# RomanBresson/KAGNN

Hardware: AMD Instinct MI355X
Metric: edges/sec KAN-GIN fwd+bwd, hidden=64 grid=5, 1M-node synthetic; HBM % peak (higher is better)
Workload: dtype f32 (fp16 hi/lo split operands, fp32 accumulate)

## Files before the change

### kagnn_amd/csrc/aggregate.hip

```cpp
#include "common.h"
#include "host.h"

namespace kagnn {


__device__ __forceinline__ float4 ld4(const float* p) { return *reinterpret_cast<const float4*>(p); }
__device__ __forceinline__ void fma4(float4& a, float w, const float4& v) {
    a.x = fmaf(w, v.x, a.x); a.y = fmaf(w, v.y, a.y); a.z = fmaf(w, v.z, a.z); a.w = fmaf(w, v.w, a.w);
}

__device__ __forceinline__ float edge_w(const AggArgs& a, int e, int j, long i) {
    float w = a.ew ? a.ew[e] : 1.0f;
    if (a.in_scale) w *= a.in_scale[j];
    if (a.skip_self && j == (int)i) w = 0.0f;
    return w;
}

__device__ __forceinline__ void stats_products(const AggArgs& a, long row, int c4, const float4& o, float4& pa, float4& pb) {
    const float4 y = ld4(a.st_y + row * a.st_ldy + c4), m = ld4(a.st_mean + c4), q = ld4(a.st_rstd + c4);
    pa = o;
    pb = make_float4(o.x * ((y.x - m.x) * q.x), o.y * ((y.y - m.y) * q.y), o.z * ((y.z - m.z) * q.z), o.w * ((y.w - m.w) * q.w));
}

template <int LPR, bool STATS, bool LEAN>
__device__ __forceinline__ void agg_rows_v4_body(const AggArgs& args) {
    AggArgs a = args;
    if constexpr (LEAN) {
        a.ew = nullptr; a.in_scale = nullptr; a.out_scale = nullptr; a.bias = nullptr; a.skip_self = 0;
        a.col_scale = nullptr; a.col_shift = nullptr;
    }
    const unsigned wg = (LEAN ? a.wg0 : 0u) + (blockIdx.x & 7) * (gridDim.x >> 3) + (blockIdx.x >> 3);
    const long gid = (wg * 256L + threadIdx.x) / LPR;
    const int c4 = (threadIdx.x % LPR) * 4;
    const bool live = gid < a.N && c4 < a.F;
    if (!STATS && !live) return;
    float4 pa = make_float4(0.f, 0.f, 0.f, 0.f), pb = pa;
    if (live) {
        const int s = a.rowptr[gid], t = a.rowptr[gid + 1];
        const bool hub = (t - s) > a.hub_threshold;
        float4 acc = ld4(a.x + gid * a.ldx + c4);
        const float sw = a.self_scale * (a.in_scale ? a.in_scale[gid] : 1.0f);
        acc.x *= sw; acc.y *= sw; acc.z *= sw; acc.w *= sw;
        if (!hub) {
            int e = s;
            for (; e + 4 <= t; e += 4) {
                const int j0 = a.col[e], j1 = a.col[e + 1], j2 = a.col[e + 2], j3 = a.col[e + 3];
                const float4 v0 = ld4(a.x + (long)j0 * a.ldx + c4);
                const float4 v1 = ld4(a.x + (long)j1 * a.ldx + c4);
                const float4 v2 = ld4(a.x + (long)j2 * a.ldx + c4);
                const float4 v3 = ld4(a.x + (long)j3 * a.ldx + c4);
                fma4(acc, edge_w(a, e, j0, gid), v0);
                fma4(acc, edge_w(a, e + 1, j1, gid), v1);
                fma4(acc, edge_w(a, e + 2, j2, gid), v2);
                fma4(acc, edge_w(a, e + 3, j3, gid), v3);
            }
            for (; e < t; ++e) {
                const int j = a.col[e];
                fma4(acc, edge_w(a, e, j, gid), ld4(a.x + (long)j * a.ldx + c4));
            }
        }
        const float os = a.out_scale ? a.out_scale[gid] : 1.0f;
        float4 b = make_float4(0.f, 0.f, 0.f, 0.f);
        if (a.bias) b = ld4(a.bias + c4);
        float4 o = make_float4(fmaf(os, acc.x, b.x), fmaf(os, acc.y, b.y), fmaf(os, acc.z, b.z), fmaf(os, acc.w, b.w));
        if (a.col_scale) {
            const float4 cs = ld4(a.col_scale + c4), ch = ld4(a.col_shift + c4);
            const float cnt = (float)(t - s) + a.self_scale;
            o.x = fmaf(cs.x, o.x, cnt * ch.x); o.y = fmaf(cs.y, o.y, cnt * ch.y);
            o.z = fmaf(cs.z, o.z, cnt * ch.z); o.w = fmaf(cs.w, o.w, cnt * ch.w);
        }
        if (a.addend && !hub) {
            const float4 d = ld4(a.addend + gid * a.lda + c4);
            o.x += d.x; o.y += d.y; o.z += d.z; o.w += d.w;
        }
        *reinterpret_cast<float4*>(a.out + gid * a.ldo + c4) = o;
        if (STATS && !hub) stats_products(a, gid, c4, o, pa, pb);
    }
    if constexpr (STATS) {
        __shared__ float4 s_a[256], s_b[256];
        s_a[threadIdx.x] = pa; s_b[threadIdx.x] = pb;
        __syncthreads();
        if (threadIdx.x < LPR && c4 < a.F && wg * 256L < a.N * LPR) {
            constexpr int R = 256 / LPR;
#pragma unroll 4
            for (int k = 1; k < R; ++k) {
                const float4 u = s_a[k * LPR + threadIdx.x], v = s_b[k * LPR + threadIdx.x];
                pa.x += u.x; pa.y += u.y; pa.z += u.z; pa.w += u.w;
                pb.x += v.x; pb.y += v.y; pb.z += v.z; pb.w += v.w;
            }
            *reinterpret_cast<float4*>(a.st_partial + (wg * 2L + 0) * a.F + c4) = pa;
            *reinterpret_cast<float4*>(a.st_partial + (wg * 2L + 1) * a.F + c4) = pb;
        }
    }
}

template <int LPR, bool STATS = false>
__global__ __launch_bounds__(256) void agg_rows_v4_kernel(AggArgs a) { agg_rows_v4_body<LPR, STATS, false>(a); }

template <int LPR>
__global__ __launch_bounds__(256) void agg_rows_v4_corun_kernel(AggArgs a) { agg_rows_v4_body<LPR, false, true>(a); }

template <int LPR>
__global__ __launch_bounds__(256) void agg_rows_ep_kernel(AggArgs a) {
    constexpr int EP = 16 / LPR;
    const long gid = (blockIdx.x * 256L + threadIdx.x) >> 4;
    const int l16 = threadIdx.x & 15, cg = l16 % LPR, eg = l16 / LPR;
    const int c4 = cg * 4;
    const bool live = gid < a.N && c4 < a.F;
    const long row = min(gid, a.N - 1);
    const int cc = live ? c4 : 0;
    const int s = a.rowptr[row], t = a.rowptr[row + 1];
    const bool hub = (t - s) > a.hub_threshold;
    float4 acc = make_float4(0.f, 0.f, 0.f, 0.f);
    if (!hub) {
        int e = s + eg;
        for (; e + EP < t; e += 2 * EP) {
            const int j0 = a.col[e], j1 = a.col[e + EP];
            const float4 v0 = ld4(a.x + (long)j0 * a.ldx + cc);
            const float4 v1 = ld4(a.x + (long)j1 * a.ldx + cc);
            fma4(acc, edge_w(a, e, j0, row), v0);
            fma4(acc, edge_w(a, e + EP, j1, row), v1);
        }
        if (e < t) {
            const int j = a.col[e];
            fma4(acc, edge_w(a, e, j, row), ld4(a.x + (long)j * a.ldx + cc));
        }
    }
#pragma unroll
    for (int o = LPR; o < 16; o <<= 1) {
        acc.x += __shfl_xor(acc.x, o); acc.y += __shfl_xor(acc.y, o);
        acc.z += __shfl_xor(acc.z, o); acc.w += __shfl_xor(acc.w, o);
    }
    if (live && eg == 0) {
        const float sw = a.self_scale * (a.in_scale ? a.in_scale[row] : 1.0f);
        const float4 xs = ld4(a.x + row * a.ldx + c4);
        const float os = a.out_scale ? a.out_scale[row] : 1.0f;
        float4 b = make_float4(0.f, 0.f, 0.f, 0.f);
        if (a.bias) b = ld4(a.bias + c4);
        float4 o = make_float4(fmaf(os, fmaf(sw, xs.x, acc.x), b.x), fmaf(os, fmaf(sw, xs.y, acc.y), b.y),
                               fmaf(os, fmaf(sw, xs.z, acc.z), b.z), fmaf(os, fmaf(sw, xs.w, acc.w), b.w));
        if (a.col_scale) {
            const float4 cs = ld4(a.col_scale + c4), ch = ld4(a.col_shift + c4);
            const float cnt = (float)(t - s) + a.self_scale;
            o.x = fmaf(cs.x, o.x, cnt * ch.x); o.y = fmaf(cs.y, o.y, cnt * ch.y);
            o.z = fmaf(cs.z, o.z, cnt * ch.z); o.w = fmaf(cs.w, o.w, cnt * ch.w);
        }
        if (a.addend && !hub) {
            const float4 d = ld4(a.addend + row * a.lda + c4);
            o.x += d.x; o.y += d.y; o.z += d.z; o.w += d.w;
        }
        *reinterpret_cast<float4*>(a.out + row * a.ldo + c4) = o;
    }
}

template <int LPR>
__global__ __launch_bounds__(256) void agg_hub_v4_kernel(AggArgs a, const int* __restrict__ seg,
                                                         float* __restrict__ part, int ldp) {
    __shared__ float4 s_part[256];
    const int row = seg[3 * blockIdx.x], e0 = seg[3 * blockIdx.x + 1], e1 = seg[3 * blockIdx.x + 2];
    constexpr int G = 256 / LPR;
    const int g = threadIdx.x / LPR, lg = threadIdx.x % LPR, c4 = lg * 4;
    float4 acc = make_float4(0.f, 0.f, 0.f, 0.f);
    if (c4 < a.F) {
        int e = e0 + g;
        for (; e + 3 * G < e1; e += 4 * G) {
            const int j0 = a.col[e], j1 = a.col[e + G], j2 = a.col[e + 2 * G], j3 = a.col[e + 3 * G];
            const float4 v0 = ld4(a.x + (long)j0 * a.ldx + c4);
            const float4 v1 = ld4(a.x + (long)j1 * a.ldx + c4);
            const float4 v2 = ld4(a.x + (long)j2 * a.ldx + c4);
            const float4 v3 = ld4(a.x + (long)j3 * a.ldx + c4);
            fma4(acc, edge_w(a, e, j0, row), v0);
            fma4(acc, edge_w(a, e + G, j1, row), v1);
            fma4(acc, edge_w(a, e + 2 * G, j2, row), v2);
            fma4(acc, edge_w(a, e + 3 * G, j3, row), v3);
        }
        for (; e < e1; e += G) {
            const int j = a.col[e];
            fma4(acc, edge_w(a, e, j, row), ld4(a.x + (long)j * a.ldx + c4));
        }
    }
    s_part[threadIdx.x] = acc;
    __syncthreads();
    if (g == 0 && c4 < a.F) {
#pragma unroll 8
        for (int k = 1; k < G; ++k) {
            const float4 p = s_part[k * LPR + lg];
            acc.x += p.x; acc.y += p.y; acc.z += p.z; acc.w += p.w;
        }
        *reinterpret_cast<float4*>(part + (long)blockIdx.x * ldp + c4) = acc;
    }
}

template <int LPR, bool STATS = false>
__global__ __launch_bounds__(256) void agg_hub_merge_kernel(AggArgs a, const int* __restrict__ seg, long nseg,
                                                            const float* __restrict__ part, int ldp, long st_row0 = 0) {
    __shared__ float4 s_part[256];
// ... 148 lines not shown
}

__global__ __launch_bounds__(256) void embedding_fwd_kernel(const int64_t* __restrict__ idx, long stride, long N,
                                                            const float* __restrict__ table, int V, int F,
                                                            float* __restrict__ out, long ldo, int accumulate) {
    const long i = blockIdx.x * 4L + (threadIdx.x >> 6);
    if (i >= N) return;
    const int lane = threadIdx.x & 63;
    const int64_t v = idx[i * stride];
    const bool ok = v >= 0 && v < V;
    for (int f = lane; f < F; f += 64) {
        const float t = ok ? table[v * F + f] : __builtin_nanf("");
        out[i * ldo + f] = accumulate ? out[i * ldo + f] + t : t;
    }
}

constexpr int kEmbRows = 128;
template <int WAVES>
__global__ __launch_bounds__(64 * WAVES) void embedding_bwd_partial_kernel(const int64_t* __restrict__ idx, long stride, long N,
                                                                           const float* __restrict__ g, long ldg, int V, int F,
                                                                           float* __restrict__ partial) {
    extern __shared__ float s_acc[];
    const int lane = threadIdx.x & 63, wave = __builtin_amdgcn_readfirstlane(threadIdx.x >> 6), f = blockIdx.y * 64 + lane;
    float* acc = s_acc + (size_t)wave * V * 64;
    for (int k = lane; k < V * 64; k += 64) acc[k] = 0.0f;
    __builtin_amdgcn_wave_barrier();
    constexpr int RPW = kEmbRows / WAVES;
    const long r0 = ((long)blockIdx.x * WAVES + wave) * RPW, r1 = min(N, r0 + RPW);
    const bool col_ok = f < F;
    const int fc = min(f, F - 1);
    for (long i0 = r0; i0 < r1; i0 += 16) {
        int64_t iv[16];
        float gv[16];
#pragma unroll
        for (int u = 0; u < 16; ++u) iv[u] = idx[min(i0 + u, r1 - 1) * stride];
#pragma unroll
        for (int u = 0; u < 16; ++u) gv[u] = g[min(i0 + u, r1 - 1) * ldg + fc];
#pragma unroll
        for (int u = 0; u < 16; ++u) {
            const bool hit = i0 + u < r1 && iv[u] >= 0 && iv[u] < V;
            const float val = col_ok ? gv[u] : 0.0f;
            if (hit) acc[(int)iv[u] * 64 + lane] += val;
        }
    }
    __syncthreads();
    for (int k = threadIdx.x; k < V * 64; k += 64 * WAVES) {
        const int v = k >> 6, ff = blockIdx.y * 64 + (k & 63);
        float a = s_acc[k];
#pragma unroll
        for (int w = 1; w < WAVES; ++w) a += s_acc[(size_t)w * V * 64 + k];
        if (ff < F) partial[((long)blockIdx.x * V + v) * F + ff] = a;
    }
}

__global__ __launch_bounds__(256) void embedding_bwd_reduce_kernel(const float* __restrict__ partial, int nb, int V, int F,
                                                                   float* __restrict__ g_table) {
    __shared__ float s_part[8][32];
    const int e = threadIdx.x & 31, sub = threadIdx.x >> 5;
    const long per = (long)V * F, k = blockIdx.x * 32L + e;
    const int chunk = (nb + 7) / 8, b0 = sub * chunk, b1 = min(nb, b0 + chunk);
    float a = 0.0f;
    if (k < per) {
        int b = b0;
        for (; b + 8 <= b1; b += 8) {
            float t[8];
#pragma unroll
            for (int u = 0; u < 8; ++u) t[u] = partial[(b + u) * per + k];
#pragma unroll
            for (int u = 0; u < 8; ++u) a += t[u];
        }
        for (; b < b1; ++b) a += partial[b * per + k];
    }
    s_part[sub][e] = a;
    __syncthreads();
    if (sub == 0 && k < per) {
        float t = s_part[0][e];
#pragma unroll
        for (int q = 1; q < 8; ++q) t += s_part[q][e];
        g_table[k] = t;
    }
}

int embedding_fwd(const int64_t* idx, long stride, long N, const float* table, int V, int F, float* out, long ldo, int accumulate,
                  hipStream_t st) {
    if (N == 0) return KAGNN_OK;
    embedding_fwd_kernel<<<cdiv(N, 4), 256, 0, st>>>(idx, stride, N, table, V, F, out, ldo, accumulate);
    KAGNN_LAUNCH_CHECK();
    return KAGNN_OK;
}

size_t embedding_bwd_ws_bytes(long N, int V, int F) { return (size_t)cdiv(max(N, 1L), kEmbRows) * V * F * sizeof(float); }

int embedding_bwd(const int64_t* idx, long stride, long N, const float* g, long ldg, int V, int F, float* g_table, float* ws,
                  size_t ws_bytes, hipStream_t st) {
    if (V == 0) return KAGNN_OK;
    if (V > 512) return fail(KAGNN_ERR_UNSUPPORTED, "%s: tables of at most 512 rows (the categorical encoders of the graph-level models)", "embedding_bwd");
    if (ws_bytes < embedding_bwd_ws_bytes(N, V, F)) return fail(KAGNN_ERR_ARG, "%s: workspace too small", "embedding_bwd");
    const size_t tbl = (size_t)V * 64 * sizeof(float);
    const int waves = 4 * tbl <= 64 * 1024 ? 4 : 2 * tbl <= 128 * 1024 ? 2 : 1;
    const int nb = cdiv(max(N, 1L), (long)kEmbRows);
    const size_t lds = waves * tbl;
    if (lds > 64 * 1024) {
        static unsigned long long configured = 0;
        if (auto first_use_ = first_use_on_this_device(configured)) {
            KAGNN_HIP(hipFuncSetAttribute((const void*)embedding_bwd_partial_kernel<1>, hipFuncAttributeMaxDynamicSharedMemorySize, 128 * 1024 + 1024));
            KAGNN_HIP(hipFuncSetAttribute((const void*)embedding_bwd_partial_kernel<2>, hipFuncAttributeMaxDynamicSharedMemorySize, 128 * 1024 + 1024));
        }
    }
    const dim3 grid((unsigned)nb, (unsigned)cdiv(F, 64));
    if (waves == 4) embedding_bwd_partial_kernel<4><<<grid, 256, lds, st>>>(idx, stride, N, g, ldg, V, F, ws);
    else if (waves == 2) embedding_bwd_partial_kernel<2><<<grid, 128, lds, st>>>(idx, stride, N, g, ldg, V, F, ws);
    else embedding_bwd_partial_kernel<1><<<grid, 64, lds, st>>>(idx, stride, N, g, ldg, V, F, ws);
    KAGNN_LAUNCH_CHECK();
    embedding_bwd_reduce_kernel<<<cdiv((long)V * F, 32), 256, 0, st>>>(ws, nb, V, F, g_table);
    KAGNN_LAUNCH_CHECK();
    return KAGNN_OK;
}

static bool vec4_ok(const AggArgs& a) {
    auto al = [](const void* p) { return (reinterpret_cast<uintptr_t>(p) & 15) == 0; };
    return a.F % 4 == 0 && a.F <= 256 && a.ldx % 4 == 0 && a.ldo % 4 == 0 && al(a.x) && al(a.out) &&
           (!a.bias || al(a.bias)) && (!a.addend || (al(a.addend) && a.lda % 4 == 0)) &&
           (!a.col_scale || (al(a.col_scale) && al(a.col_shift)));
}

size_t aggregate_ws_bytes(long num_hub_seg, int F) { return (size_t)num_hub_seg * (size_t)((F + 3) & ~3) * sizeof(float); }

int aggregate_hub_rows(const AggArgs& a, const int* hub_seg, long num_hub_seg, float* ws, size_t ws_bytes, hipStream_t st) {
    if (num_hub_seg <= 0) return KAGNN_OK;
    const int ldp = (a.F + 3) & ~3;
    if ((size_t)num_hub_seg * ldp * sizeof(float) > ws_bytes) return fail(KAGNN_ERR_ARG, "%s: workspace too small", "aggregate_hub_rows");
#define HUBS(LPR)                                                                                   \
    {                                                                                               \
        agg_hub_v4_kernel<LPR><<<(unsigned)num_hub_seg, 256, 0, st>>>(a, hub_seg, ws, ldp);         \
        KAGNN_LAUNCH_CHECK();                                                                       \
        agg_hub_merge_kernel<LPR><<<(unsigned)num_hub_seg, 256, 0, st>>>(a, hub_seg, num_hub_seg, ws, ldp); \
        KAGNN_LAUNCH_CHECK();                                                                       \
    }
    if (a.F <= 4) HUBS(1) else if (a.F <= 8) HUBS(2) else if (a.F <= 16) HUBS(4) else if (a.F <= 32) HUBS(8)
    else if (a.F <= 64) HUBS(16) else if (a.F <= 128) HUBS(32) else HUBS(64)
#undef HUBS
    return KAGNN_OK;
}

static int stats_lpr(int F) { return F <= 32 ? 8 : F <= 64 ? 16 : F <= 128 ? 32 : 64; }
bool aggregate_stats_ok(const AggArgs& a) {
    auto al = [](const void* p) { return (reinterpret_cast<uintptr_t>(p) & 15) == 0; };
    return vec4_ok(a) && a.F > 16 && a.st_y && a.st_mean && a.st_rstd && a.st_partial && a.st_ldy % 4 == 0 && al(a.st_y) &&
           al(a.st_mean) && al(a.st_rstd) && al(a.st_partial);
}
long aggregate_stats_rows(long N, int F, long num_hub_seg) { return (long)cdiv(N * stats_lpr(F), 256) + (num_hub_seg > 0 ? num_hub_seg : 0); }

bool aggregate_corun_ok(const AggArgs& a) {
    return vec4_ok(a) && a.F > 32 && a.F <= 64 && !a.ew && !a.in_scale && !a.out_scale && !a.bias && !a.skip_self && !a.col_scale && !a.st_partial;
}

int aggregate_sum(const AggArgs& a, const int* hub_seg, long num_hub_seg, float* ws, size_t ws_bytes, hipStream_t st, const AggCorun* corun) {
    if (a.N == 0) return KAGNN_OK;
    if (corun && !(aggregate_corun_ok(a) && corun->head_pct >= 0 && corun->head_pct < 100 && corun->side_done))
        return fail(KAGNN_ERR_ARG, "%s: the co-run launch does not cover this call", "aggregate_sum");
    const bool stats = a.st_partial != nullptr;
    if (stats && !aggregate_stats_ok(a)) return fail(KAGNN_ERR_UNSUPPORTED, "%s: column statistics need 16-byte aligned fp32 rows of 17..256 columns", "aggregate_sum");
    if (!vec4_ok(a)) {
        AggArgs b = a;
        b.hub_threshold = 0x7fffffff;
        dim3 grid((unsigned)a.N, cdiv(a.F, 256));
        agg_rows_generic_kernel<<<grid, 256, 0, st>>>(b);
        KAGNN_LAUNCH_CHECK();
        return KAGNN_OK;
    }
    AggArgs b = a;
    if (num_hub_seg == 0 || hub_seg == nullptr) b.hub_threshold = 0x7fffffff;
    const int ldp = (a.F + 3) & ~3;
    if (b.hub_threshold != 0x7fffffff && (ws == nullptr || ws_bytes < aggregate_ws_bytes(num_hub_seg, a.F)))
        return fail(KAGNN_ERR_ARG, "%s: workspace too small for the hub segments (see kagnn_aggregate_workspace_bytes)", "aggregate_sum");
#define HUBS(LPR, ST)                                                                               \
    if (b.hub_threshold != 0x7fffffff) {                                                            \
        agg_hub_v4_kernel<LPR><<<(unsigned)num_hub_seg, 256, 0, st>>>(b, hub_seg, ws, ldp);         \
        KAGNN_LAUNCH_CHECK();                                                                       \
        agg_hub_merge_kernel<LPR, ST><<<(unsigned)num_hub_seg, 256, 0, st>>>(b, hub_seg, num_hub_seg, ws, ldp, (long)cdiv(a.N * LPR, 256)); \
        KAGNN_LAUNCH_CHECK();                                                                       \
    }
#define AGG_ROWS_GRID(threads) (cdiv(cdiv((threads), 256), 8) * 8)
#define ROWS(LPR)                                                                     \
    {                                                                                 \
        if (stats) {                                                                  \
            agg_rows_v4_kernel<LPR, true><<<AGG_ROWS_GRID(a.N * LPR), 256, 0, st>>>(b);   \
            KAGNN_LAUNCH_CHECK();                                                     \
            HUBS(LPR, true)                                                           \
        } else {                                                                      \
            if (corun && LPR == 16) {         \
                const unsigned total = AGG_ROWS_GRID(a.N * LPR);       \
                const unsigned head = (unsigned)((unsigned long)total * (unsigned)corun->head_pct / 100) & ~7u; \
                if (head) {                                                           \
                    agg_rows_v4_corun_kernel<16><<<head, 256, kAggCorunLds, st>>>(b); \
                    KAGNN_LAUNCH_CHECK();                                             \
                }                                                                     \
                KAGNN_HIP(hipStreamWaitEvent(st, corun->side_done, 0));               \
                AggArgs t = b;                                                        \
                t.wg0 = head;                                                         \
                agg_rows_v4_corun_kernel<16><<<total - head, 256, 0, st>>>(t);        \
            } else                                                                    \
                agg_rows_v4_kernel<LPR><<<AGG_ROWS_GRID(a.N * LPR), 256, 0, st>>>(b);   \
            KAGNN_LAUNCH_CHECK();                                                     \
            HUBS(LPR, false)                                                          \
        }                                                                             \
    }
#define ROWS_EP(LPR)                                                                  \
    {                                                                                 \
        agg_rows_ep_kernel<LPR><<<cdiv(a.N * 16, 256), 256, 0, st>>>(b);              \
        KAGNN_LAUNCH_CHECK();                                                         \
        HUBS(LPR, false)                                                              \
    }
    if (a.F <= 4) ROWS_EP(1) else if (a.F <= 8) ROWS_EP(2) else if (a.F <= 16) ROWS_EP(4) else if (a.F <= 32) ROWS(8)
    else if (a.F <= 64) ROWS(16)
    else if (a.F <= 128) ROWS(32) else ROWS(64)
#undef ROWS
#undef AGG_ROWS_GRID
#undef ROWS_EP
#undef HUBS
    return KAGNN_OK;
}

int gcn_deg_inv_sqrt(const int* rowptr, const int* col, long N, float* dis, hipStream_t st) {
    if (N == 0) return KAGNN_OK;
    gcn_deg_kernel<<<cdiv(N, 256), 256, 0, st>>>(rowptr, col, N, dis);
    KAGNN_LAUNCH_CHECK();
    return KAGNN_OK;
}

int gine_fwd(const float* x, long ldx, const float* ea, long lde, float* out, long ldo,
             const int* rowptr, const int* col, const int* perm, long N, int F, float self_scale,
             hipStream_t st) {
    if (N == 0) return KAGNN_OK;
    gine_fwd_kernel<<<cdiv(N, 4), 256, 0, st>>>(x, ldx, ea, lde, out, ldo, rowptr, col, perm, N, F, self_scale);
    KAGNN_LAUNCH_CHECK();
    return KAGNN_OK;
}

int gine_bwd(const float* x, long ldx, const float* ea, long lde, const float* gout, long ldg,
             float* gx, long ldgx, float* gea, long ldge, const int* rowptr, const int* col,
             const int* perm, long N, int F, float self_scale, hipStream_t st, int gea_accumulate) {
    if (N == 0) return KAGNN_OK;
    gine_bwd_kernel<<<cdiv(N, 4), 256, 0, st>>>(x, ldx, ea, lde, gout, ldg, gx, ldgx, gea, ldge, rowptr, col, perm, N, F, self_scale, gea_accumulate);
    KAGNN_LAUNCH_CHECK();
    return KAGNN_OK;
}

int segment_pool(const float* x, long ldx, float* out, long ldo, const int* seg, long B, int F,
                 int mean, hipStream_t st) {
    if (B == 0) return KAGNN_OK;
    segment_pool_kernel<<<cdiv(B, 4), 256, 0, st>>>(x, ldx, out, ldo, seg, B, F, mean);
    KAGNN_LAUNCH_CHECK();
    return KAGNN_OK;
}

int segment_bcast(const float* g, long ldg, float* gx, long ldgx, const int* seg, long B, int F,
                  int mean, hipStream_t st) {
    if (B == 0) return KAGNN_OK;
    segment_bcast_kernel<<<cdiv(B, 4), 256, 0, st>>>(g, ldg, gx, ldgx, seg, B, F, mean);
    KAGNN_LAUNCH_CHECK();
    return KAGNN_OK;
}

}
```

### kagnn_amd/csrc/fused_calls.hip

```cpp
#include "host.h"
#include <mutex>

using namespace kagnn;

namespace {
struct GraphSide {
    const int32_t* rowptr; const int32_t* col; const int32_t* hub_seg; int64_t num_hub_seg; int32_t hub_threshold; float self_scale;
};
struct KanChain {
    int64_t N; int32_t L; const int32_t* widths;
    const float* const* bw; const float* const* sw; const float* const* sc;
    const float* const* acts; const void* const* pack_fwd; const void* const* pack_dx;
    const float* knots; int32_t G, K, mode;
};
struct LayerIn {
    const void* x; int32_t x_dtype; int64_t ldx; const float* in_col_scale; const float* in_col_shift; float* col_mean; float* col_m2;
};
struct LayerGrads {
    const float* gy; int64_t ldgy; void* gx; int32_t gx_dtype; int64_t ldgx; int32_t bf16_gather; const float* gx_addend; int64_t ld_addend;
    float* const* g_bw; float* const* g_sw; float* const* g_sc;
};

struct GineStage {
    const float* x; int64_t ldx; const float* ea; int64_t lde; const int32_t* perm;
    float* g_ea; int64_t ldge;
    int accumulate_g_ea = 0;
    int prepacked = 0;
};
struct BnStage { const float* y; int64_t ldy; const float* weight; const float* mean; const float* rstd; float* g_weight; float* g_bias; };
struct StatsOut { const float* y; int64_t ldy; const float* mean; const float* rstd; float* sums; };
struct DwPiece { unsigned char* base; DwDefer* defer; };

struct LayerLayout {
    size_t fwd_hub_bytes, fwd_scratch, fwd_scratch_bytes, fwd_fix, fwd_fix_bytes, fwd_total;
    size_t bwd_hub_bytes, dw, dw_bytes, g[2], bwd_total;
    size_t bn, bn_ws_bytes, bn_tab, bn_bytes, stats, stats_bytes, bwd_total_all;
    size_t dw_piece[8], dw_piece_bytes[8], dw_pieces_bytes;
    int wmax;
};

void layer_layout_optional(LayerLayout& y, int64_t N, int out, int f0, int64_t num_hub_seg_t) {
    y.bn = y.bwd_total;
    y.bn_ws_bytes = out ? bn_ws_bytes(N, out) : 0;
    y.bn_tab = y.bn + al256z(y.bn_ws_bytes);
    y.bn_bytes = out ? al256z(y.bn_ws_bytes) + al256z(4 * (size_t)((out + 63) & ~63) * sizeof(float)) : 0;
    y.stats = y.bn + y.bn_bytes;
    y.stats_bytes = f0 ? al256z(bn_stats_fold_bytes(aggregate_stats_rows(N, f0, num_hub_seg_t), f0)) : 0;
    y.bwd_total_all = y.stats + y.stats_bytes;
}

int layer_layout(int64_t N, int32_t L, const int32_t* widths, int32_t G, int32_t K, int32_t mode, int64_t num_hub_seg,
                 int64_t num_hub_seg_t, LayerLayout& y) {
    static const char fn[] = "kagnn_gin_kan_layer_workspace_bytes";
    size_t fw = 0, dw = 0;
    y.wmax = 0;
    for (int l = 0; l < L; ++l) {
        int rc = check_kan_dims(fn, widths[l], widths[l + 1], G, K, mode);
        if (rc) return rc;
        size_t b = 0;
        rc = (l == L - 1 ? kagnn_kan_fwd_moments_workspace_bytes : kagnn_kan_fwd_workspace_bytes)(N, widths[l], widths[l + 1], G, K, mode, &b);
        if (rc) return rc;
        fw = b > fw ? b : fw;
        rc = kagnn_kan_bwd_weight_workspace_bytes(N, widths[l], widths[l + 1], G, K, mode, &b); if (rc) return rc;
        dw = b > dw ? b : dw;
        y.dw_piece_bytes[l] = al256z(b);
        y.wmax = widths[l] > y.wmax ? widths[l] : y.wmax;
    }
    y.dw_pieces_bytes = 0;
    for (int l = L - 1; l >= 0; --l) { y.dw_piece[l] = y.dw_pieces_bytes; y.dw_pieces_bytes += y.dw_piece_bytes[l]; }
    y.fwd_hub_bytes = al256z(aggregate_bf16_ws_bytes(num_hub_seg, widths[0]));
    y.fwd_scratch = y.fwd_hub_bytes;
    y.fwd_fix = y.fwd_scratch + al256z(fw);
    y.fwd_total = y.fwd_fix + al256z(widths[0] <= 32 ? kan_sparse_fwd_agg_ws_bytes(num_hub_seg, widths[0], widths[1]) : 0) + 256;
    y.fwd_scratch_bytes = y.fwd_total - y.fwd_scratch;
    y.fwd_fix_bytes = y.fwd_total - y.fwd_fix;
    y.bwd_hub_bytes = al256z(aggregate_bf16_ws_bytes(num_hub_seg_t, widths[0]));
    y.dw = y.bwd_hub_bytes;
    y.dw_bytes = al256z(dw);
    const size_t g_bytes = al256z((size_t)N * y.wmax * sizeof(float));
    y.g[0] = y.dw + y.dw_bytes;
    y.g[1] = y.g[0] + g_bytes;
    y.bwd_total = y.g[1] + g_bytes + 256;
    layer_layout_optional(y, N, 0, 0, 0);
    return KAGNN_OK;
}

int layer_fwd_impl(const GraphSide& gr, const KanChain& c, const LayerIn& in, const GineStage* gine, void* workspace,
                   size_t workspace_bytes, void* stream, const char* fn) {
    (void)fn;
    const int64_t N = c.N;
    const int32_t L = c.L, G = c.G, K = c.K, mode = c.mode;
    const int32_t* widths = c.widths;
    float* const* acts = const_cast<float* const*>(c.acts);
    void* const* pack_fwd = const_cast<void* const*>(c.pack_fwd);
    void* const* pack_dx = const_cast<void* const*>(c.pack_dx);
    KAGNN_CHECK_ARG(N >= 0 && L >= 1 && L <= 8 && widths && c.bw && c.sw && acts && pack_fwd && pack_dx, "bad argument");
    KAGNN_CHECK_ARG((in.in_col_scale == nullptr) == (in.in_col_shift == nullptr), "in_col_scale and in_col_shift must both be given or both be null");
    KAGNN_CHECK_ARG(!in.in_col_scale || in.x_dtype == KAGNN_DTYPE_F32, "the column affine of the gathered matrix needs fp32 rows");
    KAGNN_CHECK_ARG((in.col_mean == nullptr) == (in.col_m2 == nullptr), "col_mean and col_m2 must both be given or both be null");
    LayerLayout lay;
    int rc = layer_layout(N, L, widths, G, K, mode, gr.num_hub_seg, 0, lay);
    if (rc) return rc;
    KAGNN_CHECK_ARG(workspace && workspace_bytes >= lay.fwd_total, "workspace too small (kagnn_gin_kan_layer_workspace_bytes)");
    if (N == 0) return KAGNN_OK;
    unsigned char* ws = static_cast<unsigned char*>(workspace);
    const char* fuse_e = getenv("KAGNN_FUSE_AGG");
    const bool fuse_env = fuse_e != nullptr && atoi(fuse_e) != 0;
    const bool fuse = fuse_env && !gine && !in.in_col_scale && in.x_dtype == KAGNN_DTYPE_F32 && mode == KAGNN_PREC_SPLIT && !(L == 1 && in.col_mean) &&
                      use_sparse_fwd(widths[0], widths[1], G, K, mode) &&
                      kan_sparse_fwd_agg_ok(static_cast<const float*>(in.x), in.ldx, N, widths[0], widths[1], G, K);
    if (gine)
        rc = kagnn_aggregate_gine(static_cast<const float*>(in.x), in.ldx, gine->ea, gine->lde, acts[0], widths[0], gr.rowptr, gr.col, gine->perm, N,
                                  widths[0], gr.self_scale, stream);
    else if (fuse)
        rc = KAGNN_OK;
    else if (in.x_dtype == KAGNN_DTYPE_BF16)
        rc = kagnn_aggregate_sum_bf16(in.x, in.ldx, acts[0], widths[0], KAGNN_DTYPE_F32, gr.rowptr, gr.col, nullptr, N, widths[0], gr.self_scale,
                                      nullptr, nullptr, nullptr, 0, gr.hub_seg, gr.num_hub_seg, gr.hub_threshold, ws, lay.fwd_hub_bytes, stream);
    else if (in.in_col_scale)
        rc = kagnn_aggregate_sum_affine(static_cast<const float*>(in.x), in.ldx, acts[0], widths[0], gr.rowptr, gr.col, N, widths[0], gr.self_scale,
                                        in.in_col_scale, in.in_col_shift, gr.hub_seg, gr.num_hub_seg, gr.hub_threshold, nullptr, 0, ws,
                                        lay.fwd_hub_bytes, stream);
    else
        rc = kagnn_aggregate_sum(static_cast<const float*>(in.x), in.ldx, acts[0], widths[0], gr.rowptr, gr.col, nullptr, N, widths[0],
                                 gr.self_scale, nullptr, nullptr, nullptr, 0, gr.hub_seg, gr.num_hub_seg, gr.hub_threshold, ws, lay.fwd_hub_bytes,
                                 stream);
    if (rc) return rc;
    const bool prepacked = gine && gine->prepacked;
    bool batched = L >= 2 && !prepacked;
    int in_[8], out_[8];
    for (int l = 0; l < L; ++l) {
        in_[l] = widths[l]; out_[l] = widths[l + 1];
        batched = batched && use_split_dx(in_[l], out_[l], G, K, mode) && use_sparse_fwd(in_[l], out_[l], G, K, mode) &&
                  kan_fused_pack_ok(in_[l], out_[l], G + K);
    }
    if (batched) {
        rc = kagnn_kan_pack_batch(L, c.bw, c.sw, c.sc, in_, out_, G, K, mode, pack_fwd, pack_dx, stream);
        if (rc) return rc;
    } else if (!prepacked) {
        for (int l = 0; l < L; ++l) {
            rc = kagnn_kan_pack(c.bw[l], c.sw[l], c.sc ? c.sc[l] : nullptr, in_[l], out_[l], G, K, mode, pack_fwd[l], pack_dx[l], stream);
            if (rc) return rc;
        }
    }
    for (int l = 0; l < L; ++l) {
        if (l == 0 && fuse) {
            KAGNN_STAGE_AS("kagnn_kan_linear_fwd+aggregate_sum (one kernel)", stream);
            rc = kan_sparse_fwd_agg(static_cast<const float*>(in.x), in.ldx, N, gr.rowptr, gr.col, gr.hub_seg, gr.num_hub_seg, gr.hub_threshold,
                                    gr.self_scale, c.knots, in_[0], out_[0], G, K, pack_fwd[0], acts[0], in_[0], acts[1], out_[0],
                                    ws + lay.fwd_fix, lay.fwd_fix_bytes, as_stream(stream));
            if (rc) return rc;
            continue;
        }
        if (l == L - 1 && in.col_mean)
            rc = kagnn_kan_linear_fwd_moments(acts[l], in_[l], N, c.knots, in_[l], out_[l], G, K, mode, pack_fwd[l], acts[l + 1],
                                              out_[l], in.col_mean, in.col_m2, ws + lay.fwd_scratch, lay.fwd_scratch_bytes, stream);
        else
            rc = kagnn_kan_linear_fwd(acts[l], in_[l], N, c.knots, in_[l], out_[l], G, K, mode, pack_fwd[l], acts[l + 1], out_[l],
                                      ws + lay.fwd_scratch, lay.fwd_scratch_bytes, stream);
        if (rc) return rc;
    }
    return KAGNN_OK;
}

struct BwdSide { hipStream_t stream = nullptr; hipEvent_t fork = nullptr, join = nullptr; };
constexpr int kBwdSideMaxDevices = 64;
std::mutex g_bwd_side_mu;
BwdSide g_bwd_side[kBwdSideMaxDevices];

class BwdFork {
    std::unique_lock<std::mutex> lk_;
    BwdSide* s_ = nullptr;
    hipStream_t caller_ = nullptr;
    bool forked_ = false, recorded_ = false;
public:
    BwdFork() = default;
    BwdFork(const BwdFork&) = delete;
    BwdFork& operator=(const BwdFork&) = delete;
    int prepare(hipStream_t caller) {
        int dev = 0;
        KAGNN_HIP(hipGetDevice(&dev));
        if (dev < 0 || dev >= kBwdSideMaxDevices) return fail(KAGNN_ERR_UNSUPPORTED, "%s: device index out of range", "layer_bwd");
        lk_ = std::unique_lock<std::mutex>(g_bwd_side_mu);
        BwdSide& s = g_bwd_side[dev];
        if (!s.stream) KAGNN_HIP(hipStreamCreateWithFlags(&s.stream, hipStreamNonBlocking));
        if (!s.fork) KAGNN_HIP(hipEventCreateWithFlags(&s.fork, hipEventDisableTiming));
        if (!s.join) KAGNN_HIP(hipEventCreateWithFlags(&s.join, hipEventDisableTiming));
        s_ = &s; caller_ = caller;
        return KAGNN_OK;
    }
    int fork() {
        KAGNN_HIP(hipEventRecord(s_->fork, caller_));
        KAGNN_HIP(hipStreamWaitEvent(s_->stream, s_->fork, 0));
        forked_ = true;
        return KAGNN_OK;
    }
    hipStream_t side() const { return s_->stream; }
    int side_done(hipEvent_t* ev) {
        KAGNN_HIP(hipEventRecord(s_->join, s_->stream));
        recorded_ = true;
        *ev = s_->join;
        return KAGNN_OK;
    }
    void joined() { forked_ = false; }
    int join() {
        if (!forked_) return KAGNN_OK;
        forked_ = false;
        if (!recorded_) KAGNN_HIP(hipEventRecord(s_->join, s_->stream));
        KAGNN_HIP(hipStreamWaitEvent(caller_, s_->join, 0));
        return KAGNN_OK;
    }
    ~BwdFork() { (void)join(); }
};

constexpr int kAggCorunHeadPct = 35;
bool dw_corun_ok(int in, int out, int G, int K, int mode) {
    return use_split_dw(in, out, G, K, mode) && !g_half_products && K == 3 && G + K <= 8 && in > 32 && in <= 64 && out <= 64;
}

int layer_bwd_impl(const GraphSide& gr, const KanChain& c, const LayerGrads& io, const BnStage* bn, const float* bn_sums_in,
                   const StatsOut* so, const GineStage* gine, const DwPiece* piece, void* workspace, size_t workspace_bytes, void* stream,
                   const char* fn) {
    const int64_t N = c.N;
    const int32_t L = c.L, G = c.G, K = c.K, mode = c.mode;
    const int32_t* widths = c.widths;
    const float* const* acts = c.acts;
    void* const gx = io.gx;
    KAGNN_CHECK_ARG(N >= 0 && L >= 1 && L <= 8 && widths && c.sw && acts && c.pack_dx && io.g_sw, "bad argument");
    KAGNN_CHECK_ARG(!io.gx_addend || (gx && io.gx_dtype == KAGNN_DTYPE_F32 && !io.bf16_gather && io.ld_addend >= widths[0]),
                    "gx_addend needs an fp32 gx and fp32 gather operands");
    LayerLayout lay;
    int rc = layer_layout(N, L, widths, G, K, mode, 0, gr.num_hub_seg, lay);
    if (rc) return rc;
    layer_layout_optional(lay, N, bn ? widths[L] : 0, so ? widths[0] : 0, gr.num_hub_seg);
    KAGNN_CHECK_ARG(!so || (so->y && so->mean && so->rstd && so->sums && so->ldy >= widths[0] && gx && io.gx_dtype == KAGNN_DTYPE_F32 && !io.bf16_gather),
                    "the previous norm's statistics need its input, mean, rstd and an fp32 gx");
    KAGNN_CHECK_ARG(!bn_sums_in || bn, "bn_sums belongs to the BatchNorm stage");
    if (!(workspace && workspace_bytes >= lay.bwd_total_all))
        return fail(KAGNN_ERR_ARG, bn ? "%s: workspace too small (kagnn_gin_kan_layer_workspace_bytes + kagnn_gin_kan_layer_bwd_bn_workspace_bytes)"
                                      : "%s: workspace too small (kagnn_gin_kan_layer_workspace_bytes)", fn);
    if (N == 0) return KAGNN_OK;
    unsigned char* ws = static_cast<unsigned char*>(workspace);
    const int wmax = lay.wmax;
    unsigned char* gbuf[2] = {ws + lay.g[0], ws + lay.g[1]};
    auto dw_on = [&](void* st, int l, const float* g, long ldg) {
        unsigned char* area = piece ? piece->base + lay.dw_piece[l] : ws + lay.dw;
        const size_t bytes = piece ? lay.dw_piece_bytes[l] : lay.dw_bytes;
        return kan_linear_bwd_weight(acts[l], widths[l], nullptr, g, ldg, N, c.knots, widths[l], widths[l + 1], G, K, mode, c.sw[l],
                                     c.sc ? c.sc[l] : nullptr, io.g_bw ? io.g_bw[l] : nullptr, io.g_sw[l], io.g_sc ? io.g_sc[l] : nullptr,
                                     area, bytes, st, piece ? piece->defer : nullptr);
    };
    BwdFork side;
    struct { int l; const float* g; long ldg; } deferred[2];
    int n_deferred = 0;
    bool overlap = false;
    if (gx && !gine && !piece && !so && !io.bf16_gather && io.gx_dtype == KAGNN_DTYPE_F32 && dw_corun_ok(widths[0], widths[1], G, K, mode)) {
        const char* env = getenv("KAGNN_BWD_OVERLAP");
        const AggArgs probe{reinterpret_cast<const float*>(gbuf[0]), widths[0], static_cast<float*>(gx), io.ldgx, gr.rowptr, gr.col, nullptr, N,
                            widths[0], gr.self_scale, nullptr, nullptr, nullptr, 0, 0x7fffffff, io.gx_addend, io.ld_addend};
        const bool gx_in_ws = static_cast<unsigned char*>(gx) + (size_t)N * io.ldgx * sizeof(float) > ws &&
                              static_cast<unsigned char*>(gx) < ws + workspace_bytes;
        overlap = (env == nullptr || atoi(env) != 0) && io.ldgx >= widths[0] && (!io.gx_addend || io.ld_addend >= widths[0]) && !gx_in_ws &&
                  aggregate_corun_ok(probe);
        if (overlap) {
            hipStreamCaptureStatus cap = hipStreamCaptureStatusNone;
            if (hipStreamIsCapturing(as_stream(stream), &cap) != hipSuccess) { (void)hipGetLastError(); overlap = false; }
            else overlap = cap == hipStreamCaptureStatusNone;
        }
        if (overlap) { rc = side.prepare(as_stream(stream)); if (rc) return rc; }
    }
    auto dw = [&](int l, const float* g, long ldg) {
        const bool alive = l == 0 || (l == L - 1 && !bn);
        if (overlap && alive && dw_corun_ok(widths[l], widths[l + 1], G, K, mode)) {
            deferred[n_deferred++] = {l, g, ldg};
            return (int)KAGNN_OK;
        }
        return dw_on(stream, l, g, ldg);
    };
    const float* g = io.gy;
    long ldg = io.ldgy;
    int cur = 0;
    bool gh0_bf16 = false;
    bool bn_in_dx = false;
    BnBack bnb{};
    if (bn) {
        const int out = widths[L], ldt = (out + 63) & ~63;
        KAGNN_CHECK_ARG(bn->y && bn->mean && bn->rstd && bn->ldy >= out && N >= 2, "bad BatchNorm stage");
        unsigned char* bws = ws + lay.bn;
        float* tab = reinterpret_cast<float*>(ws + lay.bn_tab);
        bnb = BnBack{bn->y, (long)bn->ldy, tab, ldt, reinterpret_cast<float*>(gbuf[1]), (long)out};
        const int in = widths[L - 1];
        bn_in_dx = mode == KAGNN_PREC_SPLIT && use_split_dx(in, out, G, K, mode) && out <= wmax && !(L == 1 && (gx == nullptr || io.bf16_gather)) &&
                   fits32(N, ldg) && kan_split_dx_bn_ok(ldg, in, out, G, K, bnb, g);
        if (bn_in_dx && bn_sums_in) {
            KAGNN_STAGE_AS("kagnn_batchnorm_bwd statistics given (in ..._layer_bwd_bn)", stream);
            rc = bn_bwd_stats_given(bn_sums_in, N, out, bn->weight, bn->mean, bn->rstd, bn->g_weight, bn->g_bias, tab, ldt, as_stream(stream));
            if (rc) return rc;
        } else if (bn_in_dx) {
            KAGNN_STAGE_AS("kagnn_batchnorm_bwd statistics (in ..._layer_bwd_bn)", stream);
            rc = bn_bwd_stats(bn->y, bn->ldy, g, ldg, N, out, bn->weight, bn->mean, bn->rstd, bn->g_weight, bn->g_bias, tab, ldt, bws,
                              lay.bn_ws_bytes, as_stream(stream));
            if (rc) return rc;
        } else {
            if (out > wmax) return fail(KAGNN_ERR_UNSUPPORTED, "%s: a BatchNorm stage wider than every layer input is not covered", fn);
            KAGNN_STAGE_AS("kagnn_batchnorm_bwd", stream);
            rc = bn_bwd(bn->y, bn->ldy, g, ldg, N, out, bn->weight, bn->mean, bn->rstd, 1, 0.0f, 0ULL, reinterpret_cast<float*>(gbuf[1]), out,
                        bn->g_weight, bn->g_bias, bws, lay.bn_ws_bytes, as_stream(stream));
            if (rc) return rc;
            g = reinterpret_cast<const float*>(gbuf[1]); ldg = out;
        }
    }
    for (int l = L - 1; l >= 0; --l) {
        const int in = widths[l], out = widths[l + 1];
        const bool fused_bn = bn_in_dx && l == L - 1;
        if (fused_bn) {
            {
                KAGNN_STAGE_AS("kagnn_kan_linear_bwd_input", stream);
                rc = kan_split_dx_bn(acts[l], in, g, ldg, N, c.knots, in, out, G, K, c.pack_dx[l], reinterpret_cast<float*>(gbuf[0]), in, bnb,
                                     as_stream(stream));
            }
            if (rc) return rc;
            rc = dw(l, bnb.gy_out, bnb.ldo);
            if (rc) return rc;
            if (l == 0 && gx == nullptr) break;
            g = reinterpret_cast<const float*>(gbuf[0]); ldg = in; cur = 1;
            continue;
        }
        rc = dw(l, g, ldg);
        if (rc) return rc;
        if (l == 0 && gx == nullptr) break;
        const bool b16 = l == 0 && io.bf16_gather && mode == KAGNN_PREC_SPLIT && K == 3 && G + K <= 8 && out <= 128 && in % 8 == 0 &&
                         in <= 512  &&
                         use_split_dx(in, out, G, K, mode);
        rc = kagnn_kan_linear_bwd_input(acts[l], in, g, ldg, N, c.knots, in, out, G, K, mode, c.pack_dx[l], gbuf[cur], in,
                                        b16 ? KAGNN_DTYPE_BF16 : KAGNN_DTYPE_F32, stream);
        if (rc) return rc;
        g = reinterpret_cast<const float*>(gbuf[cur]); ldg = in; cur ^= 1;
        gh0_bf16 = b16;
    }
    if (gx == nullptr) return KAGNN_OK;
    const int f0 = widths[0];
    if (overlap) {
        rc = side.fork();
        if (rc) return rc;
        for (int k = 0; k < n_deferred; ++k) {
            rc = dw_on(side.side(), deferred[k].l, deferred[k].g, deferred[k].ldg);
            if (rc) return rc;
        }
        const AggArgs a{g, ldg, static_cast<float*>(gx), io.ldgx, gr.rowptr, gr.col, nullptr, N, f0, gr.self_scale, nullptr, nullptr, nullptr,
                        0, gr.hub_threshold > 0 ? gr.hub_threshold : 0x7fffffff, io.gx_addend, io.ld_addend};
        AggCorun corun{kAggCorunHeadPct * n_deferred, nullptr};
        rc = side.side_done(&corun.side_done);
        if (rc) return rc;
        KAGNN_STAGE_AS("kagnn_aggregate_sum", stream);
        rc = aggregate_sum(a, gr.hub_seg, gr.num_hub_seg, reinterpret_cast<float*>(ws), lay.bwd_hub_bytes, as_stream(stream), &corun);
        if (rc) return rc;
        side.joined();
        return KAGNN_OK;
    }
    if (gine)
        return gine_bwd(gine->x, gine->ldx, gine->ea, gine->lde, g, ldg, static_cast<float*>(gx), io.ldgx, gine->g_ea, gine->ldge,
                        gr.rowptr, gr.col, gine->perm, N, f0, gr.self_scale, as_stream(stream), gine->accumulate_g_ea);
    if (gh0_bf16 || io.gx_dtype == KAGNN_DTYPE_BF16) {
        const void* src = g;
        if (!gh0_bf16) {
            rc = kagnn_rows_to_bf16(g, ldg, gbuf[cur], f0, N, f0, stream);
            if (rc) return rc;
            src = gbuf[cur];
        }
        return kagnn_aggregate_sum_bf16(src, f0, gx, io.ldgx, io.gx_dtype, gr.rowptr, gr.col, nullptr, N, f0, gr.self_scale, nullptr, nullptr,
                                        nullptr, 0, gr.hub_seg, gr.num_hub_seg, gr.hub_threshold, ws, lay.bwd_hub_bytes, stream);
    }
    if (so) {
        AggArgs a{g, ldg, static_cast<float*>(gx), io.ldgx, gr.rowptr, gr.col, nullptr, N, f0, gr.self_scale, nullptr, nullptr, nullptr,
                  0, gr.hub_threshold > 0 ? gr.hub_threshold : 0x7fffffff, io.gx_addend, io.ld_addend};
        float* partial = reinterpret_cast<float*>(ws + lay.stats);
        a.st_y = so->y; a.st_ldy = so->ldy; a.st_mean = so->mean; a.st_rstd = so->rstd; a.st_partial = partial;
        KAGNN_CHECK_ARG(ldg >= f0 && io.ldgx >= f0 && (!io.gx_addend || io.ld_addend >= f0), "leading dimension smaller than num_feat");
        if (!aggregate_stats_ok(a)) return fail(KAGNN_ERR_UNSUPPORTED, "%s: the previous norm's statistics need 17..256 input features in 16-byte aligned fp32 rows", fn);
        {
            KAGNN_STAGE_AS("kagnn_aggregate_sum", stream);
            rc = aggregate_sum(a, gr.hub_seg, gr.num_hub_seg, reinterpret_cast<float*>(ws), lay.bwd_hub_bytes, as_stream(stream));
            if (rc) return rc;
        }
        KAGNN_STAGE_AS("kagnn_batchnorm_bwd statistics fold", stream);
        const bool hubs = gr.num_hub_seg > 0 && gr.hub_seg != nullptr && gr.hub_threshold > 0;
        return bn_sums_from_partials(partial, aggregate_stats_rows(N, f0, hubs ? gr.num_hub_seg : 0), f0, so->sums, as_stream(stream));
    }
    return kagnn_aggregate_sum_add(g, ldg, static_cast<float*>(gx), io.ldgx, gr.rowptr, gr.col, nullptr, N, f0, gr.self_scale, nullptr,
                                   nullptr, nullptr, 0, gr.hub_seg, gr.num_hub_seg, gr.hub_threshold, io.gx_addend, io.ld_addend, ws,
                                   lay.bwd_hub_bytes, stream);
}

struct StackLayout {
    LayerLayout layer;
    size_t fwd_layer_bytes, bn_ws, bn_ws_bytes, moments, fwd_total;
    size_t bwd_layer_bytes, pp[2], arena, arena_conv_bytes, arena_bytes, bwd_total;
};

int stack_layout(int64_t N, int32_t nconv, int32_t L, const int32_t* widths, int32_t G, int32_t K, int32_t mode, StackLayout& s) {
    int rc = layer_layout(N, L, widths, G, K, mode, 0, 0, s.layer);
    if (rc) return rc;
    layer_layout_optional(s.layer, N, widths[L], 0, 0);
    s.fwd_layer_bytes = al256z(s.layer.fwd_total);
    s.bn_ws = s.fwd_layer_bytes;
    s.bn_ws_bytes = bn_ws_bytes(N, widths[L]);
    s.moments = s.bn_ws + al256z(s.bn_ws_bytes);
    s.fwd_total = s.moments + al256z(2 * (size_t)widths[L] * sizeof(float)) + 256;
    s.bwd_layer_bytes = al256z(s.layer.bwd_total_all);
    const size_t g_bytes = al256z((size_t)N * widths[0] * sizeof(float));
    s.pp[0] = s.bwd_layer_bytes;
    s.pp[1] = s.pp[0] + g_bytes;
    s.arena = s.pp[1] + g_bytes;
    s.arena_conv_bytes = nconv * L <= kDwDeferMax ? s.layer.dw_pieces_bytes : 0;
    s.arena_bytes = s.arena_conv_bytes * (size_t)nconv;
    s.bwd_total = s.arena + s.arena_bytes + 256;
    return KAGNN_OK;
}

int stack_fwd_impl(const float* x, int64_t ldx, const float* edge_attr, int64_t lde, int64_t N, const int32_t* rowptr,
                   const int32_t* col, const int32_t* perm, const float* self_scale, int32_t nconv,
                   int32_t L, const int32_t* widths, const float* const* bw, const float* const* sw,
                   const float* const* sc, const float* knots, int32_t G, int32_t K, int32_t mode,
                   float* const* acts, void* const* pack_fwd, void* const* pack_dx,
                   const float* const* bn_weight, const float* const* bn_bias, float* const* running_mean,
                   float* const* running_var, const float* momentum, const float* eps,
                   float* const* h, float* const* save_mean, float* const* save_rstd,
                   void* workspace, size_t workspace_bytes, void* stream, bool prepacked) {
    static const char fn[] = "kagnn_gine_kan_stack_fwd";
    ModeScope mode_scope_(mode);
    KAGNN_CHECK_ARG_AS(fn, nconv >= 1 && L >= 1 && L <= 8 && widths && self_scale && bw && sw && acts && pack_fwd && pack_dx && bn_weight && bn_bias &&
                       momentum && eps && h && save_mean && save_rstd, "null array");
    KAGNN_CHECK_ARG_AS(fn, widths[0] == widths[L] && N >= 2, "hidden -> hidden chains, at least two rows (batch statistics)");
    StackLayout lay;
    int rc = stack_layout(N, nconv, L, widths, G, K, mode, lay);
    if (rc) return rc;
    KAGNN_CHECK_ARG_AS(fn, workspace && workspace_bytes >= lay.fwd_total, "workspace too small (kagnn_gine_kan_stack_workspace_bytes)");
    unsigned char* ws = static_cast<unsigned char*>(workspace);
    float* mom = reinterpret_cast<float*>(ws + lay.moments);
    const int H = widths[L];
    int in_[16], out_[16];
    bool batch = nconv * L <= 16;
    for (int k = 0; k < nconv * L && batch; ++k) {
        in_[k] = widths[k % L]; out_[k] = widths[k % L + 1];
        batch = use_split_dx(in_[k], out_[k], G, K, mode) && use_sparse_fwd(in_[k], out_[k], G, K, mode) && kan_fused_pack_ok(in_[k], out_[k], G + K);
    }
    if (batch && !prepacked) { rc = kagnn_kan_pack_batch(nconv * L, bw, sw, sc, in_, out_, G, K, mode, pack_fwd, pack_dx, stream); if (rc) return rc; }
    const float* in = x;
    int64_t ldin = ldx;
    for (int i = 0; i < nconv; ++i) {
        GineStage gs{in, ldin, edge_attr, lde, perm, nullptr, 0};
        gs.prepacked = batch ? 1 : 0;
        const GraphSide gr{.rowptr = rowptr, .col = col, .self_scale = self_scale[i]};
        const KanChain c{.N = N, .L = L, .widths = widths, .bw = bw + i * L, .sw = sw + i * L, .sc = sc ? sc + i * L : nullptr,
                         .acts = acts + i * (L + 1), .pack_fwd = pack_fwd + i * L, .pack_dx = pack_dx + i * L, .knots = knots, .G = G, .K = K,
                         .mode = mode};
        const LayerIn li{.x = in, .x_dtype = KAGNN_DTYPE_F32, .ldx = ldin, .col_mean = mom,
                         .col_m2 = mom + H};
        rc = layer_fwd_impl(gr, c, li, &gs, ws, lay.fwd_layer_bytes, stream, fn);
        if (rc) return rc;
        rc = kagnn_batchnorm_fwd(acts[i * (L + 1) + L], H, N, H, bn_weight[i], bn_bias[i], running_mean ? running_mean[i] : nullptr,
                                 running_var ? running_var[i] : nullptr, momentum[i], eps[i], 1, mom, mom + H, 0.0f, 0ULL, h[i], H,
                                 save_mean[i], save_rstd[i], ws + lay.bn_ws, lay.bn_ws_bytes, stream);
        if (rc) return rc;
        in = h[i]; ldin = H;
    }
    return KAGNN_OK;
}
}

#pragma GCC visibility push(default)
extern "C" {

int kagnn_gin_kan_layer_workspace_bytes(int64_t N, int32_t L, const int32_t* widths, int32_t G, int32_t K, int32_t mode,
                                        int64_t num_hub_seg, int64_t num_hub_seg_t, size_t* fwd_bytes, size_t* bwd_bytes) {
    ModeScope mode_scope_(mode);
    KAGNN_CHECK_ARG(N >= 0 && L >= 1 && L <= 8 && widths && fwd_bytes && bwd_bytes, "bad argument");
    LayerLayout lay;
    int rc = layer_layout(N, L, widths, G, K, mode, num_hub_seg, num_hub_seg_t, lay);
    if (rc) return rc;
    *fwd_bytes = lay.fwd_total;
    *bwd_bytes = lay.bwd_total;
    return KAGNN_OK;
}

int kagnn_gin_kan_layer_fwd(const void* x, int32_t x_dtype, int64_t ldx, int64_t N, const int32_t* rowptr, const int32_t* col,
                            const int32_t* hub_seg, int64_t num_hub_seg, int32_t hub_threshold, float self_scale,
                            int32_t L, const int32_t* widths, const float* const* bw, const float* const* sw,
                            const float* const* sc, const float* knots, int32_t G, int32_t K, int32_t mode,
                            float* const* acts, void* const* pack_fwd, void* const* pack_dx, float* col_mean,
                            float* col_m2, void* workspace, size_t workspace_bytes, void* stream) {
    ModeScope mode_scope_(mode);
    const GraphSide gr{.rowptr = rowptr, .col = col, .hub_seg = hub_seg, .num_hub_seg = num_hub_seg, .hub_threshold = hub_threshold,
                       .self_scale = self_scale};
    const KanChain c{.N = N, .L = L, .widths = widths, .bw = bw, .sw = sw, .sc = sc, .acts = acts, .pack_fwd = pack_fwd, .pack_dx = pack_dx,
                     .knots = knots, .G = G, .K = K, .mode = mode};
    const LayerIn in{.x = x, .x_dtype = x_dtype, .ldx = ldx, .col_mean = col_mean, .col_m2 = col_m2};
    return layer_fwd_impl(gr, c, in, nullptr, workspace, workspace_bytes, stream, __func__);
}

int kagnn_gin_kan_layer_fwd_affine(const float* x, int64_t ldx, int64_t N, const int32_t* rowptr, const int32_t* col,
                                   const int32_t* hub_seg, int64_t num_hub_seg, int32_t hub_threshold, float self_scale,
                                   const float* in_col_scale, const float* in_col_shift,
                                   int32_t L, const int32_t* widths, const float* const* bw, const float* const* sw,
// ... 512 lines not shown
```

Measured before the change: 4.572 billion.

## Software-pipeline lean neighbor gather and raise aggregate co-run head share

Adds a dedicated gather loop for the lean aggregation path. It prefetches the next group of column indices while the current rows load, uses asm barriers to keep loads issued in order, and uses 32-bit byte-offset addressing. The point is to hide index-load latency and trim the address arithmetic in the memory-bound SpMM gather. The co-run head fraction also goes from 35 to 50 percent, capped at 100, and the tail launch is skipped when the head covers everything. That moves more aggregation work to run alongside the deferred weight-gradient kernels, but it risks contention with the side stream.

```diff
diff --git a/kagnn_amd/csrc/aggregate.hip b/kagnn_amd/csrc/aggregate.hip
--- a/kagnn_amd/csrc/aggregate.hip
+++ b/kagnn_amd/csrc/aggregate.hip
@@ -20,6 +20,39 @@
     const float4 y = ld4(a.st_y + row * a.st_ldy + c4), m = ld4(a.st_mean + c4), q = ld4(a.st_rstd + c4);
     pa = o;
     pb = make_float4(o.x * ((y.x - m.x) * q.x), o.y * ((y.y - m.y) * q.y), o.z * ((y.z - m.z) * q.z), o.w * ((y.w - m.w) * q.w));
+}
+
+__device__ __forceinline__ void add4(float4& a, const float4& v) { a.x += v.x; a.y += v.y; a.z += v.z; a.w += v.w; }
+__device__ __forceinline__ void lean_gather(float4& acc, const float* xc, unsigned ldb, const int* __restrict__ col, int s, int t) {
+    auto row = [&](int j) { return *reinterpret_cast<const float4*>(reinterpret_cast<const char*>(xc) + (unsigned long)(unsigned)j * ldb); };
+    if (s >= t) return;
+    const int* cp = col + s;
+    int n = (t - s) >> 2;
+    const int r = (t - s) & 3;
+    int j0 = 0, j1 = 0, j2 = 0, j3 = 0;
+    if (n > 0) { j0 = cp[0]; j1 = cp[1]; j2 = cp[2]; j3 = cp[3]; }
+    else { j0 = cp[0]; if (r > 1) j1 = cp[1]; if (r > 2) j2 = cp[2]; }
+    while (n > 0) {
+        const float4 v0 = row(j0);
+        asm volatile("" : "+v"(j1) : : "memory");
+        const float4 v1 = row(j1);
+        asm volatile("" : "+v"(j2) : : "memory");
+        const float4 v2 = row(j2);
+        asm volatile("" : "+v"(j3) : : "memory");
+        const float4 v3 = row(j3);
+        asm volatile("" : : : "memory");
+        cp += 4;
+        --n;
+        if (n > 0) { j0 = cp[0]; j1 = cp[1]; j2 = cp[2]; j3 = cp[3]; }
+        else if (r > 0) { j0 = cp[0]; if (r > 1) j1 = cp[1]; if (r > 2) j2 = cp[2]; }
+        add4(acc, v0); add4(acc, v1); add4(acc, v2); add4(acc, v3);
+    }
+    const float4 none = make_float4(-0.0f, -0.0f, -0.0f, -0.0f);
+    float4 v0 = none, v1 = none, v2 = none;
+    if (r > 0) v0 = row(j0);
+    if (r > 1) v1 = row(j1);
+    if (r > 2) v2 = row(j2);
+    add4(acc, v0); add4(acc, v1); add4(acc, v2);
 }
 
 template <int LPR, bool STATS, bool LEAN>
@@ -41,7 +74,9 @@
         float4 acc = ld4(a.x + gid * a.ldx + c4);
         const float sw = a.self_scale * (a.in_scale ? a.in_scale[gid] : 1.0f);
         acc.x *= sw; acc.y *= sw; acc.z *= sw; acc.w *= sw;
-        if (!hub) {
+        if constexpr (LEAN) {
+            if (!hub) lean_gather(acc, a.x + c4, (unsigned)a.ldx * 4u, a.col, s, t);
+        } else if (!hub) {
             int e = s;
             for (; e + 4 <= t; e += 4) {
                 const int j0 = a.col[e], j1 = a.col[e + 1], j2 = a.col[e + 2], j3 = a.col[e + 3];
@@ -496,12 +531,13 @@
 long aggregate_stats_rows(long N, int F, long num_hub_seg) { return (long)cdiv(N * stats_lpr(F), 256) + (num_hub_seg > 0 ? num_hub_seg : 0); }
 
 bool aggregate_corun_ok(const AggArgs& a) {
-    return vec4_ok(a) && a.F > 32 && a.F <= 64 && !a.ew && !a.in_scale && !a.out_scale && !a.bias && !a.skip_self && !a.col_scale && !a.st_partial;
+    return vec4_ok(a) && a.F > 32 && a.F <= 64 && !a.ew && !a.in_scale && !a.out_scale && !a.bias && !a.skip_self && !a.col_scale && !a.st_partial &&
+           a.ldx < (1L << 30);
 }
 
 int aggregate_sum(const AggArgs& a, const int* hub_seg, long num_hub_seg, float* ws, size_t ws_bytes, hipStream_t st, const AggCorun* corun) {
     if (a.N == 0) return KAGNN_OK;
-    if (corun && !(aggregate_corun_ok(a) && corun->head_pct >= 0 && corun->head_pct < 100 && corun->side_done))
+    if (corun && !(aggregate_corun_ok(a) && corun->head_pct >= 0 && corun->head_pct <= 100 && corun->side_done))
         return fail(KAGNN_ERR_ARG, "%s: the co-run launch does not cover this call", "aggregate_sum");
     const bool stats = a.st_partial != nullptr;
     if (stats && !aggregate_stats_ok(a)) return fail(KAGNN_ERR_UNSUPPORTED, "%s: column statistics need 16-byte aligned fp32 rows of 17..256 columns", "aggregate_sum");
@@ -541,9 +577,11 @@
                     KAGNN_LAUNCH_CHECK();                                             \
                 }                                                                     \
                 KAGNN_HIP(hipStreamWaitEvent(st, corun->side_done, 0));               \
-                AggArgs t = b;                                                        \
-                t.wg0 = head;                                                         \
-                agg_rows_v4_corun_kernel<16><<<total - head, 256, 0, st>>>(t);        \
+                if (head < total) {           \
+                    AggArgs t = b;                                                    \
+                    t.wg0 = head;                                                     \
+                    agg_rows_v4_corun_kernel<16><<<total - head, 256, 0, st>>>(t);    \
+                }                                                                     \
             } else                                                                    \
                 agg_rows_v4_kernel<LPR><<<AGG_ROWS_GRID(a.N * LPR), 256, 0, st>>>(b);   \
             KAGNN_LAUNCH_CHECK();                                                     \
diff --git a/kagnn_amd/csrc/fused_calls.hip b/kagnn_amd/csrc/fused_calls.hip
--- a/kagnn_amd/csrc/fused_calls.hip
+++ b/kagnn_amd/csrc/fused_calls.hip
@@ -1,4 +1,5 @@
 #include "host.h"
+#include <algorithm>
 #include <mutex>
 
 using namespace kagnn;
@@ -213,7 +214,7 @@
     ~BwdFork() { (void)join(); }
 };
 
-constexpr int kAggCorunHeadPct = 35;
+constexpr int kAggCorunHeadPct = 50;
 bool dw_corun_ok(int in, int out, int G, int K, int mode) {
     return use_split_dw(in, out, G, K, mode) && !g_half_products && K == 3 && G + K <= 8 && in > 32 && in <= 64 && out <= 64;
 }
@@ -349,7 +350,7 @@
         }
         const AggArgs a{g, ldg, static_cast<float*>(gx), io.ldgx, gr.rowptr, gr.col, nullptr, N, f0, gr.self_scale, nullptr, nullptr, nullptr,
                         0, gr.hub_threshold > 0 ? gr.hub_threshold : 0x7fffffff, io.gx_addend, io.ld_addend};
-        AggCorun corun{kAggCorunHeadPct * n_deferred, nullptr};
+        AggCorun corun{std::min(100, kAggCorunHeadPct * n_deferred), nullptr};
         rc = side.side_done(&corun.side_done);
         if (rc) return rc;
         KAGNN_STAGE_AS("kagnn_aggregate_sum", stream);
```

Result: faster. 4.766 billion, median of 6 (+4.2%).
